# daigo0927/tf-raft

Measured on NVIDIA H100. Metric: frame-pairs/sec at 448×512 iters=12; final-flow max-abs vs ref, higher is better.
Workload: dtype f32

## Files before the change

tf_raft_b200/csrc/conv_tc.cuh:

```cuda
#pragma once
#include "common.cuh"
#include "kernels.cuh"
#include "tmap.cuh"

namespace raft {

enum TcEpilogue : int {
  EPI_LINEAR = 0,
  EPI_GRU_ZR = 1,
  EPI_GRU_Q = 2,
};
enum TcAct : int { ACT_NONE = 0, ACT_RELU = 1 };

constexpr int kTileM = 128;
constexpr int kChunkK = 64;
constexpr int kABytes = kTileM * kChunkK * 2;
constexpr int kMaxTileN = 128;
constexpr int kConsumerWGs = 2;
constexpr int kConsumerWarps = 4 * kConsumerWGs;
constexpr int kTcThreads = 128 * kConsumerWGs + 128;
constexpr int kStageCols = 64;
constexpr int kStagingBytes = kConsumerWGs * 64 * kStageCols * 4;
constexpr int kSmemMax = 227 * 1024;
constexpr int kSmemFixed = 1024  + kStagingBytes + 512 ;

struct alignas(64) TcConvParams {
  CUtensorMap a_map[2];
  CUtensorMap b_map;
  int nseg, seg_chunks[2], seg_c0[2];
  int kh, kw, ph, pw;
  int stride;
  int B, H, W, TH, TW, tiles_x, tiles_y;
  int bn, n_total;
  int n_tiles_n;
  int nstages, stage_bytes;
  int group_chunks;
  int mode, act;
  const float* bias;
  const float* inv_scale;
  float out_scale;
  float* out_f32; int f32_stride, f32_c0;
  __half* out_hi; __half* out_lo; int h_stride, h_c0;
  const float* post_scale;
  const float* post_shift;
  const float* residual; int res_stride, res_c0;
  const float* concat_src; int concat_n;
  float* z; int hid;
  float* h;
  float* adv_coords;
  float* adv_flow;
};

#if defined(__CUDA_ARCH__)
__device__ __forceinline__ float4 ld4(const float* p) { return *reinterpret_cast<const float4*>(p); }
__device__ __forceinline__ float4 ldg4(const float* p) { return __ldg(reinterpret_cast<const float4*>(p)); }
__device__ __forceinline__ void st4(float* p, float4 v) { *reinterpret_cast<float4*>(p) = v; }
__device__ __forceinline__ void st8u(void* p, const uint32_t (&r)[8]) {
  reinterpret_cast<uint4*>(p)[0] = make_uint4(r[0], r[1], r[2], r[3]);
  reinterpret_cast<uint4*>(p)[1] = make_uint4(r[4], r[5], r[6], r[7]);
}
__device__ __forceinline__ void ldcg8(const float* p, float (&r)[8]) {
  const float4 a = __ldcg(reinterpret_cast<const float4*>(p)), b = __ldcg(reinterpret_cast<const float4*>(p) + 1);
  r[0] = a.x; r[1] = a.y; r[2] = a.z; r[3] = a.w; r[4] = b.x; r[5] = b.y; r[6] = b.z; r[7] = b.w;
}
__device__ __forceinline__ void ldnc8(const float* p, float (&r)[8]) {
  const float4 a = __ldg(reinterpret_cast<const float4*>(p)), b = __ldg(reinterpret_cast<const float4*>(p) + 1);
  r[0] = a.x; r[1] = a.y; r[2] = a.z; r[3] = a.w; r[4] = b.x; r[5] = b.y; r[6] = b.z; r[7] = b.w;
}
__device__ __forceinline__ void st8f(float* p, float a, float b, float c, float d, float e, float f, float g, float h) {
  const uint32_t r[8] = {__float_as_uint(a), __float_as_uint(b), __float_as_uint(c), __float_as_uint(d),
                         __float_as_uint(e), __float_as_uint(f), __float_as_uint(g), __float_as_uint(h)};
  st8u(p, r);
}
__device__ __forceinline__ float4 ldcg4(const float* p) { return __ldcg(reinterpret_cast<const float4*>(p)); }

__device__ __forceinline__ float fast_sigmoid(float x) { return __fdividef(1.0f, 1.0f + __expf(-x)); }
__device__ __forceinline__ float fast_tanh(float x) { return 1.0f - __fdividef(2.0f, 1.0f + __expf(2.0f * x)); }

template <int MODE>
__device__ __forceinline__ void tc_epilogue_regs(const TcConvParams& p, float (&v)[32], size_t pix, int col, int ncol,
                                                 float inv_scale) {
  if (p.bias) {
#pragma unroll
    for (int q = 0; q < 8; ++q) {
      const float4 bq = ldg4(p.bias + col + 4 * q);
      v[4 * q] = v[4 * q] * inv_scale + bq.x; v[4 * q + 1] = v[4 * q + 1] * inv_scale + bq.y;
      v[4 * q + 2] = v[4 * q + 2] * inv_scale + bq.z; v[4 * q + 3] = v[4 * q + 3] * inv_scale + bq.w;
    }
  } else {
#pragma unroll
    for (int j = 0; j < 32; ++j) v[j] *= inv_scale;
  }
  if (MODE == EPI_LINEAR && p.post_scale) {
#pragma unroll
    for (int q = 0; q < 8; ++q) {
      const float4 sc = ldg4(p.post_scale + col + 4 * q), sh = ldg4(p.post_shift + col + 4 * q);
      v[4 * q] = v[4 * q] * sc.x + sh.x; v[4 * q + 1] = v[4 * q + 1] * sc.y + sh.y;
      v[4 * q + 2] = v[4 * q + 2] * sc.z + sh.z; v[4 * q + 3] = v[4 * q + 3] * sc.w + sh.w;
    }
  }

  __half* dhi = nullptr;
  __half* dlo = nullptr;
  if (MODE == EPI_LINEAR) {
    const bool full = col + 32 <= p.n_total;
// ... 119 lines not shown

  if (dhi) {
    const bool wide = ((reinterpret_cast<uintptr_t>(dhi) | reinterpret_cast<uintptr_t>(dlo)) & 31) == 0;
#pragma unroll
    for (int q = 0; q < 2; ++q) {
      uint32_t ph[8], pl[8];
#pragma unroll
      for (int e = 0; e < 8; ++e) split_f16x2(v[16 * q + 2 * e], v[16 * q + 2 * e + 1], ph[e], pl[e]);
      if (wide) {
        st8u(dhi + 16 * q, ph);
        st8u(dlo + 16 * q, pl);
      } else {
        reinterpret_cast<uint4*>(dhi)[2 * q] = make_uint4(ph[0], ph[1], ph[2], ph[3]);
        reinterpret_cast<uint4*>(dhi)[2 * q + 1] = make_uint4(ph[4], ph[5], ph[6], ph[7]);
        reinterpret_cast<uint4*>(dlo)[2 * q] = make_uint4(pl[0], pl[1], pl[2], pl[3]);
        reinterpret_cast<uint4*>(dlo)[2 * q + 1] = make_uint4(pl[4], pl[5], pl[6], pl[7]);
      }
    }
  }
}

struct RingPos {
  int slot;
  uint32_t par;
};

__device__ __forceinline__ int ring_next(RingPos& r, int nst) {
  const int s = r.slot;
  r.slot = s + 1 == nst ? 0 : s + 1;
  return s;
}

__device__ __forceinline__ void ring_init(uint64_t* full_bar, uint64_t* empty_bar, int nst) {
  for (int s = 0; s < nst; ++s) {
    mbar_init(&full_bar[s], 1);
    mbar_init(&empty_bar[s], kConsumerWarps);
  }
}

struct RingSlot {
  uint8_t* data;
  uint64_t* full;
};

__device__ __forceinline__ RingSlot ring_acquire(uint8_t* stages, const int& slot_bytes, const int& nst, uint64_t* full_bar,
                                                 uint64_t* empty_bar, RingPos& rp, const int& tx) {
  const int s = ring_next(rp, nst);
  mbar_wait(&empty_bar[s], ((rp.par >> s) & 1u) ^ 1u);
  rp.par ^= 1u << s;
  mbar_arrive_expect_tx(&full_bar[s], (uint32_t)tx);
  return RingSlot{stages + (size_t)s * slot_bytes, &full_bar[s]};
}

template <int N>
__device__ __forceinline__ void ring_mma(float (&racc)[N / 2], uint8_t* stages, const int& slot_bytes, const int& nst,
                                         uint64_t* full_bar, uint64_t* empty_bar, RingPos& rp, int wg, uint32_t b_lo_off,
                                         int total, const int& group_chunks) {
  const int lane = threadIdx.x & 31;
  float acc[N / 2];
#pragma unroll
  for (int i = 0; i < N / 2; ++i) acc[i] = racc[i] = 0.0f;
  for (int done = 0; done < total;) {
    const int gend = min(total, done + group_chunks);
    for (int first = 1; done < gend; ++done, first = 0) {
      const int s = ring_next(rp, nst);
      mbar_wait(&full_bar[s], (rp.par >> s) & 1u);
      rp.par ^= 1u << s;
      const uint32_t sa = smem_u32(stages + (size_t)s * slot_bytes);
      const uint32_t arow = (uint32_t)wg * 64 * 128;
      wgmma_fence_regs(acc);
      wgmma_fence();
      wgmma_chunk3<N>(acc, make_desc_sw128(sa + arow), make_desc_sw128(sa + kABytes + arow), make_desc_sw128(sa + 2 * kABytes),
                      make_desc_sw128(sa + 2 * kABytes + b_lo_off), first != 0);
      wgmma_commit();
      wgmma_wait_all();
      wgmma_fence_regs(acc);
      __syncwarp();
      if (lane == 0) mbar_arrive(&empty_bar[s]);
    }
#pragma unroll
    for (int i = 0; i < N / 2; ++i) racc[i] += acc[i];
  }
}

__device__ __forceinline__ int tc_total_chunks(const TcConvParams& c) {
  return c.kh * c.kw * (c.seg_chunks[0] + (c.nseg > 1 ? c.seg_chunks[1] : 0));
}

__device__ __forceinline__ void tc_produce_tile(const TcConvParams& c, uint8_t* stages, uint64_t* full_bar, uint64_t* empty_bar,
                                                RingPos& rp, int nt, int b, int ty, int tx, unsigned int* next_item = nullptr,
                                                int* claim = nullptr) {
  const int ntaps = c.kh * c.kw;
  const int x0 = tx * c.TW * c.stride, y0 = ty * c.TH * c.stride, n0 = nt * c.bn;
  int left = tc_total_chunks(c);
  for (int tap = 0; tap < ntaps; ++tap) {
    const int dy = tap / c.kw - c.ph, dx = tap % c.kw - c.pw;
    int kc = 0;
    for (int seg = 0; seg < c.nseg; ++seg) {
      for (int ch = 0; ch < c.seg_chunks[seg]; ++ch, ++kc) {
        if (--left == 0 && claim) *claim = (int)atomicAdd(next_item, 1u);
        const RingSlot st = ring_acquire(stages, c.stage_bytes, c.nstages, full_bar, empty_bar, rp, c.stage_bytes);
        tma_load_5d(st.data, &c.a_map[seg], st.full, c.seg_c0[seg] + ch * kChunkK, x0 + dx, y0 + dy, b, 0);
        tma_load_4d(st.data + 2 * kABytes, &c.b_map, st.full, kc * kChunkK, n0, tap, 0);
      }
    }
  }
}

__device__ __forceinline__ int stg_idx(int r, int c) { return r * kStageCols + ((((c >> 2) ^ (r & 7))) << 2) + (c & 3); }

template <int N>
__device__ __forceinline__ void tc_consume_tile(const TcConvParams& c, uint8_t* stages, float* staging, uint64_t* full_bar,
                                                uint64_t* empty_bar, RingPos& rp, int wg, int tid, int nt, int b, int ty,
                                                int tx) {
  const int lane = tid & 31, w = tid >> 5;
  float racc[N / 2];
  ring_mma<N>(racc, stages, c.stage_bytes, c.nstages, full_bar, empty_bar, rp, wg, (uint32_t)(c.bn * kChunkK * 2),
              tc_total_chunks(c), c.group_chunks);

  float* stg = staging + wg * 64 * kStageCols;
  const int row = tid & 63, half = tid >> 6;
  const int m = wg * 64 + row;
  const int x = tx * c.TW + m % c.TW, y = ty * c.TH + m / c.TW;
  const bool inside = x < c.W && y < c.H;
  const size_t pix = ((size_t)b * c.H + y) * c.W + x;
  const float inv_scale = c.inv_scale ? __ldg(c.inv_scale) : 1.0f;
#pragma unroll
  for (int cb = 0; cb < (N + kStageCols - 1) / kStageCols; ++cb) {
    if (cb * kStageCols >= c.bn) break;
    wg_sync(wg);
#pragma unroll
    for (int i = cb * 8; i < min(cb * 8 + 8, N / 8); ++i) {
      const int col = 8 * (i - cb * 8) + 2 * (lane & 3), r0 = 16 * w + (lane >> 2);
      *reinterpret_cast<float2*>(stg + stg_idx(r0, col)) = make_float2(racc[4 * i], racc[4 * i + 1]);
      *reinterpret_cast<float2*>(stg + stg_idx(r0 + 8, col)) = make_float2(racc[4 * i + 2], racc[4 * i + 3]);
    }
    wg_sync(wg);
    const int c0 = cb * kStageCols + half * 32;
    if (inside && c0 < c.bn) {
      const int ncol = min(32, c.bn - c0);
      float v[32];
#pragma unroll
      for (int q = 0; q < 8; ++q) {
        const float4 t4 = *reinterpret_cast<const float4*>(stg + stg_idx(row, half * 32 + 4 * q));
        v[4 * q] = t4.x; v[4 * q + 1] = t4.y; v[4 * q + 2] = t4.z; v[4 * q + 3] = t4.w;
      }
#pragma unroll
      for (int j = 0; j < 32; ++j)
        if (j >= ncol) v[j] = 0.0f;
      if (c.mode == EPI_LINEAR) tc_epilogue_regs<EPI_LINEAR>(c, v, pix, nt * c.bn + c0, ncol, inv_scale);
      else if (c.mode == EPI_GRU_ZR) tc_epilogue_regs<EPI_GRU_ZR>(c, v, pix, nt * c.bn + c0, ncol, inv_scale);
      else tc_epilogue_regs<EPI_GRU_Q>(c, v, pix, nt * c.bn + c0, ncol, inv_scale);
    }
  }
}

template <class F>
__device__ __forceinline__ void with_mma_n(int bn, F&& f) {
  if (bn <= 16) f(std::integral_constant<int, 16>{});
  else if (bn <= 32) f(std::integral_constant<int, 32>{});
  else if (bn <= 64) f(std::integral_constant<int, 64>{});
  else if (bn <= 96) f(std::integral_constant<int, 96>{});
  else f(std::integral_constant<int, 128>{});
}

__device__ __forceinline__ void regs_producer() { asm volatile("setmaxnreg.dec.sync.aligned.u32 40;\n" ::: "memory"); }
__device__ __forceinline__ void regs_consumer() { asm volatile("setmaxnreg.inc.sync.aligned.u32 232;\n" ::: "memory"); }

__device__ __forceinline__ void tc_decode_tile(const TcConvParams& c, int t, int& nt, int& b, int& ty, int& tx) {
  const int mtiles = c.B * c.tiles_y * c.tiles_x;
  nt = t / mtiles;
  int mt = t - nt * mtiles;
  tx = mt % c.tiles_x;
  mt /= c.tiles_x;
  ty = mt % c.tiles_y;
  b = mt / c.tiles_y;
}
#endif

__global__ void __launch_bounds__(kTcThreads, 1) conv_tc_kernel(const __grid_constant__ TcConvParams p) {
#if defined(__CUDA_ARCH__)
  extern __shared__ uint8_t smem_raw[];
  uint8_t* smem = reinterpret_cast<uint8_t*>((reinterpret_cast<uintptr_t>(smem_raw) + 1023) & ~uintptr_t(1023));
  const int nst = p.nstages;
  uint8_t* stages = smem;
  float* staging = reinterpret_cast<float*>(stages + (size_t)nst * p.stage_bytes);
  uint64_t* full_bar = reinterpret_cast<uint64_t*>(reinterpret_cast<uint8_t*>(staging) + kStagingBytes);
  uint64_t* empty_bar = full_bar + nst;

  const int warp = threadIdx.x >> 5;
  const int mtiles = p.B * p.tiles_y * p.tiles_x;
  const int ntiles = mtiles * p.n_tiles_n;

  if (threadIdx.x == 0) {
    ring_init(full_bar, empty_bar, nst);
    fence_mbar_init();
  }
  if (warp == kConsumerWarps && (threadIdx.x & 31) == 0) {
    prefetch_tmap(&p.a_map[0]);
    prefetch_tmap(&p.b_map);
    if (p.nseg > 1) prefetch_tmap(&p.a_map[1]);
  }
  __syncthreads();
  asm volatile("griddepcontrol.wait;" ::: "memory");
  asm volatile("griddepcontrol.launch_dependents;" ::: "memory");

  RingPos rp{0, 0u};
  if (warp >= kConsumerWarps) {
    regs_producer();
    if (warp == kConsumerWarps && elect_one()) {
      for (int t = blockIdx.x; t < ntiles; t += gridDim.x) {
        int nt, b, ty, tx;
        tc_decode_tile(p, t, nt, b, ty, tx);
        tc_produce_tile(p, stages, full_bar, empty_bar, rp, nt, b, ty, tx);
      }
    }
  } else {
    regs_consumer();
    const int wg = warp >> 2, tid = threadIdx.x & 127;
    with_mma_n(p.bn, [&](auto n) {
      for (int t = blockIdx.x; t < ntiles; t += gridDim.x) {
        int nt, b, ty, tx;
        tc_decode_tile(p, t, nt, b, ty, tx);
        tc_consume_tile<decltype(n)::value>(p, stages, staging, full_bar, empty_bar, rp, wg, tid, nt, b, ty, tx);
      }
    });
  }
#endif
}

inline void tc_pick_tile(int W, int H, int* tw, int* th) {
  long best = -1;
  for (int t = 128; t >= 8; t >>= 1) {
    const int hh = 128 / t;
    const long area = (long)round_up(W, t) * round_up(H, hh);
    if (best < 0 || area < best) {
      best = area;
      *tw = t;
      *th = hh;
    }
  }
}

inline int tc_n_split(int bn) {
  const int f = ceil_div(bn, kMaxTileN);
  return bn % (16 * f) == 0 ? f : 0;
}

inline int tc_finalize(TcConvParams& p) {
  p.tiles_x = ceil_div(p.W, p.TW);
  p.tiles_y = ceil_div(p.H, p.TH);
  p.stage_bytes = 2 * kABytes + 2 * p.bn * kChunkK * 2;
  int nst = (kSmemMax - kSmemFixed) / p.stage_bytes;
  if (nst > 8) nst = 8;
  p.nstages = nst;
  return nst * p.stage_bytes + kSmemFixed;
}

inline int tc_check(const TcConvParams& p) {
  if (p.bn % 16 != 0 || p.bn < 16 || p.bn > kMaxTileN || p.TW * p.TH != kTileM) return RAFT_ERR_BAD_SHAPE;
  if (p.mode != EPI_LINEAR && p.mode != EPI_GRU_ZR && p.mode != EPI_GRU_Q) return RAFT_ERR_UNSUPPORTED;
  if (p.group_chunks < 1) return RAFT_ERR_BAD_ARG;
  return RAFT_OK;
}

template <auto Kernel>
inline int persistent_grid(int smem, long items, unsigned* grid) {
  static int num_sms[64] = {0};
  int dev = 0;
  RAFT_CUDA_TRY(cudaGetDevice(&dev));
  int& sms = num_sms[dev & 63];
  if (!sms) {
    RAFT_CUDA_TRY(cudaFuncSetAttribute(Kernel, cudaFuncAttributeMaxDynamicSharedMemorySize, smem));
    RAFT_CUDA_TRY(cudaDeviceGetAttribute(&sms, cudaDevAttrMultiProcessorCount, dev));
  }
  *grid = (unsigned)(items < sms ? items : sms);
  return RAFT_OK;
}

inline int tc_launch(TcConvParams& p, int n_tiles_n, cudaStream_t stream) {
  RAFT_TRY(tc_check(p));
  if (p.stride < 1) p.stride = 1;
  const int smem = tc_finalize(p);
  if (p.nstages < 2) return RAFT_ERR_UNSUPPORTED;
  p.n_tiles_n = n_tiles_n;
  unsigned grid = 0;
  RAFT_TRY(persistent_grid<conv_tc_kernel>(kSmemMax, (long)p.B * p.tiles_y * p.tiles_x * n_tiles_n, &grid));
  cudaLaunchConfig_t cfg;
  memset(&cfg, 0, sizeof(cfg));
  cfg.gridDim = dim3(grid);
  cfg.blockDim = dim3((unsigned)kTcThreads);
  cfg.dynamicSmemBytes = (size_t)smem;
  cfg.stream = stream;
  cudaLaunchAttribute attr[1];
  attr[0].id = cudaLaunchAttributeProgrammaticStreamSerialization;
  attr[0].val.programmaticStreamSerializationAllowed = 1;
  cfg.attrs = attr;
  cfg.numAttrs = 1;
  ++g_launches;
  RAFT_CUDA_TRY(cudaLaunchKernelEx(&cfg, conv_tc_kernel, p));
  return raft_launch_status();
}

struct TcWeightSlot {
  size_t hi, lo, bias, scale, absmax;
  int kh, kw, cin_pad, cout_pad;
};

inline TcWeightSlot tc_weight_slot(size_t& off, int kh, int kw, int cin_pad, int cout_pad) {
  auto take = [&](size_t bytes) { const size_t o = off; off = align_up(off + bytes, 256); return o; };
  TcWeightSlot s;
  s.kh = kh; s.kw = kw; s.cin_pad = cin_pad; s.cout_pad = cout_pad;
  const size_t plane = (size_t)kh * kw * cout_pad * cin_pad * sizeof(__half);
  s.hi = take(plane);
  s.lo = take(plane);
// ... 56 lines not shown
```

tf_raft_b200/csrc/encoder.cuh:

```cuda
#pragma once
#include <algorithm>

#include "lookup.cuh"
#include "update.cuh"

namespace raft {

enum { NORM_NONE = 0, NORM_INSTANCE = 1, NORM_BATCH = 2 };

struct EncSpec { int c0; int c[3]; int s[3]; };
inline EncSpec enc_spec(int variant) {
  if (variant == RAFT_VARIANT_BASIC) return {64, {64, 96, 128}, {1, 2, 2}};
  return {32, {32, 64, 96}, {1, 2, 2}};
}
inline int pad64(int c) { return round_up(c, 64); }

struct EncNormSlot { size_t gamma, beta, fscale, fshift; int C; };
struct EncLayout {
  TcWeightSlot conv1;
  EncNormSlot norm1;
  TcWeightSlot bc1[6], bc2[6], bds[6];
  EncNormSlot bn1[6], bn2[6], bnd[6];
  int has_ds[6], bc[6], bstride[6];
  TcWeightSlot conv2;
// ... 12 lines not shown
    n.C = C;
    n.gamma = take(sizeof(float) * (C + 64)); n.beta = take(sizeof(float) * (C + 64));
    n.fscale = take(sizeof(float) * (C + 64)); n.fshift = take(sizeof(float) * (C + 64));
    return n;
  };
  L.conv1 = conv_slot(1, 1, 147, S.c0);
  L.norm1 = norm_slot(S.c0);
  int cin = S.c0;
  for (int k = 0; k < 6; ++k) {
    const int c = S.c[k / 2], st = (k % 2 == 0) ? S.s[k / 2] : 1;
    L.bc[k] = c; L.bstride[k] = st;
    L.bc1[k] = conv_slot(3, 3, cin, c);
    L.bc2[k] = conv_slot(3, 3, c, c);
    L.bn1[k] = norm_slot(c);
    L.bn2[k] = norm_slot(c);
    L.has_ds[k] = st != 1;
    if (L.has_ds[k]) { L.bds[k] = conv_slot(1, 1, cin, c); L.bnd[k] = norm_slot(c); }
    cin = c;
  }
  L.conv2 = conv_slot(1, 1, cin, out_dim);
  L.total = off;
  return L;
}

struct EncWs {
  float *X32, *O32, *Y32, *D32;
  __half *Xh, *Xl, *Oh, *Ol, *Fh, *Fl, *Ih, *Il;
  float *part, *mean, *mult;
  size_t total;
};
constexpr int kNormSplit = 64;
inline EncWs enc_ws_layout(void* base, int variant, int N, int H, int W) {
  EncWs E;
  memset(&E, 0, sizeof(E));
  const EncSpec S = enc_spec(variant);
  size_t max32 = 0, max16 = 0;
  for (int l = 0; l < 3; ++l) {
    const int d = 2 << l;
    const size_t np = (size_t)N * ((H + d - 1) / d) * ((W + d - 1) / d);
    const int c = l == 0 ? (S.c0 > S.c[0] ? S.c0 : S.c[0]) : S.c[l];
    if (np * c > max32) max32 = np * c;
    if (np * pad64(c) > max16) max16 = np * pad64(c);
  }
  uint8_t* b8 = reinterpret_cast<uint8_t*>(base);
  size_t off = 0;
  auto take = [&](size_t bytes) { uint8_t* p = b8 + off; off = align_up(off + bytes, 1024); return p; };
  E.X32 = (float*)take(max32 * 4); E.O32 = (float*)take(max32 * 4);
  E.Y32 = (float*)take(max32 * 4); E.D32 = (float*)take(max32 * 4);
  E.Xh = (__half*)take(max16 * 2); E.Xl = (__half*)take(max16 * 2);
  E.Oh = (__half*)take(max16 * 2); E.Ol = (__half*)take(max16 * 2);
  E.Fh = (__half*)take(max16 * 2); E.Fl = (__half*)take(max16 * 2);
  {
    const size_t np1 = (size_t)N * ((H + 1) / 2) * ((W + 1) / 2);
    E.Ih = (__half*)take(np1 * 192 * 2); E.Il = (__half*)take(np1 * 192 * 2);
  }
  E.part = (float*)take((size_t)N * kNormSplit * 3 * 256 * 4);
  E.mean = (float*)take((size_t)N * 256 * 4);
  E.mult = (float*)take((size_t)N * 256 * 4);
  E.total = off;
  return E;
}

inline int enc_pack_conv(const raft_conv& cv, int kh, int kw, int cin, int cout, const TcWeightSlot& s, bool flatten,
                         uint8_t* base, cudaStream_t st) {
  if (!cv.kernel || !cv.bias) return RAFT_ERR_BAD_ARG;
  if (cv.kh != kh || cv.kw != kw || cv.cin != cin || cv.cout != cout) return RAFT_ERR_BAD_SHAPE;
  const raft_conv* src[1] = {&cv};
  return tc_pack_weights(base, s, src, 1, nullptr, flatten, st);
}

inline int enc_pack_norm(const raft_norm& nm, const EncNormSlot& s, int norm_type, uint8_t* base, cudaStream_t st) {
  if (norm_type == NORM_NONE) return 0;
  if (!nm.gamma || !nm.beta) return RAFT_ERR_BAD_ARG;
  float* g = reinterpret_cast<float*>(base + s.gamma);
  float* b = reinterpret_cast<float*>(base + s.beta);
  RAFT_CUDA_TRY(cudaMemcpyAsync(g, nm.gamma, s.C * sizeof(float), cudaMemcpyDeviceToDevice, st));
  RAFT_CUDA_TRY(cudaMemcpyAsync(b, nm.beta, s.C * sizeof(float), cudaMemcpyDeviceToDevice, st));
  if (norm_type == NORM_BATCH) {
    if (!nm.moving_mean || !nm.moving_variance) return RAFT_ERR_BAD_ARG;
    return launch(bn_fold_kernel, ceil_div(s.C, 128), 128, 0, st, nm.gamma, nm.beta, nm.moving_mean, nm.moving_variance,
                  1e-3f, s.C, reinterpret_cast<float*>(base + s.fscale), reinterpret_cast<float*>(base + s.fshift));
  }
  return raft_launch_status();
}

inline int encoder_prepare(int variant, int norm_type, int out_dim, const raft_encoder_weights* w, void* prepared,
                           size_t bytes, cudaStream_t st) {
  const EncLayout L = enc_layout(variant, out_dim);
  if (L.total > bytes) return RAFT_ERR_WORKSPACE;
  const EncSpec S = enc_spec(variant);
  uint8_t* base = reinterpret_cast<uint8_t*>(prepared);
  RAFT_CUDA_TRY(cudaMemsetAsync(base, 0, L.total, st));
  RAFT_TRY(enc_pack_conv(w->conv1, 7, 7, 3, S.c0, L.conv1, true, base, st));
  RAFT_TRY(enc_pack_norm(w->norm1, L.norm1, norm_type, base, st));
  int cin = S.c0;
  for (int k = 0; k < 6; ++k) {
    const int c = L.bc[k];
    RAFT_TRY(enc_pack_conv(w->block[k].conv1, 3, 3, cin, c, L.bc1[k], false, base, st));
    RAFT_TRY(enc_pack_conv(w->block[k].conv2, 3, 3, c, c, L.bc2[k], false, base, st));
    RAFT_TRY(enc_pack_norm(w->block[k].norm1, L.bn1[k], norm_type, base, st));
    RAFT_TRY(enc_pack_norm(w->block[k].norm2, L.bn2[k], norm_type, base, st));
    if (L.has_ds[k]) {
      RAFT_TRY(enc_pack_conv(w->block[k].downsample, 1, 1, cin, c, L.bds[k], false, base, st));
      RAFT_TRY(enc_pack_norm(w->block[k].downsample_norm, L.bnd[k], norm_type, base, st));
    }
    cin = c;
  }
  RAFT_TRY(enc_pack_conv(w->conv2, 1, 1, cin, out_dim, L.conv2, false, base, st));
  return raft_launch_status();
}

struct EncCtx {
  const uint8_t* prep; EncLayout L; EncWs W; cudaStream_t st;
  int N, norm_type, stats;
  int per_image;
};

inline int enc_norm_apply(const EncCtx& c, const EncNormSlot& ns, const float* y, size_t npix, int P, int relu,
                          const float* skip32, const __half* skip_hi, const __half* skip_lo, float* out32, __half* hi,
                          __half* lo) {
  const int C = ns.C, G = c.per_image ? c.N : 1;
  const int Pg = c.per_image ? P : (int)npix;
  const float* gamma = reinterpret_cast<const float*>(c.prep + ns.gamma);
  const float* beta = reinterpret_cast<const float*>(c.prep + ns.beta);
  RAFT_TRY(launch(norm_stats_kernel, dim3((unsigned)G, kNormSplit), 256, 0, c.st, y, Pg, C, kNormSplit, c.W.part));
  RAFT_TRY(launch(norm_final_kernel, ceil_div(G * C * 32, 256), 256, 0, c.st, c.W.part, G, C, kNormSplit, gamma, 1e-3f,
                  c.W.mean, c.W.mult));
  return launch(norm_apply_kernel, grid_for(npix * (pad64(C) / 8)), 256, 0, c.st, y, npix, P, C, c.per_image, c.W.mean,
                c.W.mult, beta, relu, skip32, skip_hi, skip_lo, out32, hi, lo, pad64(C));
}

inline int enc_conv_tc(const EncCtx& c, const TcWeightSlot& cs, int cout, const EncNormSlot* ns, const __half* ahi,
                       const __half* alo, int Hin, int Win, int Hout, int Wout, int stride, int relu, const float* skip,
                       float* out32, __half* ohi, __half* olo) {
  TcConvParams p;
  memset(&p, 0, sizeof(p));
  int tw, th;
  tc_pick_tile(Wout, Hout, &tw, &th);
  if (tw * stride > 256) tw = 128 / stride, th = 128 / tw;
  const int nsplit = tc_n_split(cs.cout_pad);
  if (!nsplit) return RAFT_ERR_BAD_SHAPE;
  RAFT_TRY(make_tmap_act2(&p.a_map[0], ahi, alo, c.N, Hin, Win, cs.cin_pad, tw, th, stride));
  RAFT_TRY(tc_use_weights(p, c.prep, cs, cs.cout_pad / nsplit));
  p.nseg = 1; p.seg_chunks[0] = cs.cin_pad / kChunkK; p.seg_c0[0] = 0;
  p.stride = stride;
  if (stride == 1) { p.ph = (cs.kh - 1) / 2; p.pw = (cs.kw - 1) / 2; }
  else {
    const int tot_h = (Hout - 1) * stride + cs.kh - Hin, tot_w = (Wout - 1) * stride + cs.kw - Win;
    p.ph = (tot_h > 0 ? tot_h : 0) / 2; p.pw = (tot_w > 0 ? tot_w : 0) / 2;
  }
  p.B = c.N; p.H = Hout; p.W = Wout; p.TH = th; p.TW = tw;
  p.n_total = cout;
  p.mode = EPI_LINEAR; p.out_scale = 1.0f;
  p.out_f32 = out32; p.f32_stride = cout; p.f32_c0 = 0;
  p.out_hi = ohi; p.out_lo = olo; p.h_stride = pad64(cout); p.h_c0 = 0;
  if (ns && !c.stats && c.norm_type == NORM_BATCH) {
    p.post_scale = reinterpret_cast<const float*>(c.prep + ns->fscale);
    p.post_shift = reinterpret_cast<const float*>(c.prep + ns->fshift);
  }
  const bool fused = !(ns && c.stats);
  if (fused) {
    p.act = relu ? ACT_RELU : ACT_NONE;
    p.residual = skip; p.res_stride = cout; p.res_c0 = 0;
  } else {
    p.act = ACT_NONE; p.out_hi = nullptr; p.out_lo = nullptr;
  }
  p.group_chunks = 5;
  return tc_launch(p, nsplit, c.st);
}

inline int encoder_forward(int variant, int norm_type, int out_dim, const void* prepared, const float* images, int N,
                           int H, int W, int training, int image_norm, float* out, void* ws, size_t ws_bytes, cudaStream_t st) {
  EncCtx c;
  c.prep = reinterpret_cast<const uint8_t*>(prepared);
  c.L = enc_layout(variant, out_dim);
  c.W = enc_ws_layout(ws, variant, N, H, W);
  if (c.W.total > ws_bytes) return RAFT_ERR_WORKSPACE;
  c.st = st; c.N = N; c.norm_type = norm_type;
  c.stats = (norm_type == NORM_INSTANCE) || (norm_type == NORM_BATCH && training);
  c.per_image = norm_type == NORM_INSTANCE;
  const EncSpec S = enc_spec(variant);
  const EncLayout& L = c.L;
  const EncWs& E = c.W;

  int h = (H + 1) / 2, w = (W + 1) / 2;
  {
    const size_t npix = (size_t)N * h * w;
    const int tot_h = (h - 1) * 2 + 7 - H, tot_w = (w - 1) * 2 + 7 - W;
    const float* src = images;
    if (image_norm) {
      const size_t nimg = (size_t)N * H * W * 3;
      RAFT_TRY(launch(image_norm_kernel, grid_for(nimg), 256, 0, st, images, E.O32, nimg));
      src = E.O32;
    }
    RAFT_TRY(launch(stem_im2col_kernel, grid_for(npix * 24), 256, 0, st, src, N, H, W, h, w, (tot_h > 0 ? tot_h : 0) / 2,
                    (tot_w > 0 ? tot_w : 0) / 2, 0, E.Ih, E.Il));
    if (!c.stats && pad64(S.c0) != S.c0) {
      RAFT_CUDA_TRY(cudaMemsetAsync(E.Xh, 0, npix * pad64(S.c0) * 2, st));
      RAFT_CUDA_TRY(cudaMemsetAsync(E.Xl, 0, npix * pad64(S.c0) * 2, st));
    }
    RAFT_TRY(enc_conv_tc(c, L.conv1, S.c0, &L.norm1, E.Ih, E.Il, h, w, h, w, 1, 1, nullptr, c.stats ? E.Y32 : E.X32, E.Xh, E.Xl));
    if (c.stats) RAFT_TRY(enc_norm_apply(c, L.norm1, E.Y32, npix, h * w, 1, nullptr, nullptr, nullptr, nullptr, E.Xh, E.Xl));
  }

  float *X32 = E.X32, *O32 = E.O32;
  __half *Xh = E.Xh, *Xl = E.Xl, *Oh = E.Oh, *Ol = E.Ol;
  for (int k = 0; k < 6; ++k) {
    const int st2 = L.bstride[k], cc = L.bc[k];
    const int ho = (h + st2 - 1) / st2, wo = (w + st2 - 1) / st2;
    const size_t npo = (size_t)N * ho * wo;
    const bool zero_pad_out = pad64(cc) != cc;
    if (!c.stats && zero_pad_out) {
      RAFT_CUDA_TRY(cudaMemsetAsync(E.Fh, 0, npo * pad64(cc) * 2, st));
      RAFT_CUDA_TRY(cudaMemsetAsync(E.Fl, 0, npo * pad64(cc) * 2, st));
      RAFT_CUDA_TRY(cudaMemsetAsync(Oh, 0, npo * pad64(cc) * 2, st));
      RAFT_CUDA_TRY(cudaMemsetAsync(Ol, 0, npo * pad64(cc) * 2, st));
    }
    RAFT_TRY(enc_conv_tc(c, L.bc1[k], cc, &L.bn1[k], Xh, Xl, h, w, ho, wo, st2, 1, nullptr, c.stats ? E.Y32 : nullptr, E.Fh, E.Fl));
    if (c.stats) RAFT_TRY(enc_norm_apply(c, L.bn1[k], E.Y32, npo, ho * wo, 1, nullptr, nullptr, nullptr, nullptr, E.Fh, E.Fl));
    const float* skip = X32;
    if (L.has_ds[k]) {
      RAFT_TRY(enc_conv_tc(c, L.bds[k], cc, &L.bnd[k], Xh, Xl, h, w, ho, wo, st2, 0, nullptr, c.stats ? E.Y32 : E.D32, nullptr, nullptr));
      if (c.stats) RAFT_TRY(enc_norm_apply(c, L.bnd[k], E.Y32, npo, ho * wo, 0, nullptr, nullptr, nullptr, E.D32, nullptr, nullptr));
      skip = E.D32;
    }
    RAFT_TRY(enc_conv_tc(c, L.bc2[k], cc, &L.bn2[k], E.Fh, E.Fl, ho, wo, ho, wo, 1, 1, skip, c.stats ? E.Y32 : O32, Oh, Ol));
    if (c.stats) {
      if (L.has_ds[k]) RAFT_TRY(enc_norm_apply(c, L.bn2[k], E.Y32, npo, ho * wo, 1, E.D32, nullptr, nullptr, nullptr, Oh, Ol));
      else RAFT_TRY(enc_norm_apply(c, L.bn2[k], E.Y32, npo, ho * wo, 1, nullptr, Xh, Xl, nullptr, Oh, Ol));
    }
    float* t32 = X32; X32 = O32; O32 = t32;
    __half* th_ = Xh; Xh = Oh; Oh = th_;
    __half* tl_ = Xl; Xl = Ol; Ol = tl_;
    h = ho; w = wo;
  }
  RAFT_TRY(enc_conv_tc(c, L.conv2, out_dim, nullptr, Xh, Xl, h, w, h, w, 1, 0, nullptr, out, nullptr, nullptr));
  return raft_launch_status();
}

}
```

tf_raft_b200/csrc/kernels.cuh:

```cuda
#pragma once
#include "common.cuh"

namespace raft {

__global__ void split_plane_kernel(const float* __restrict__ src, int src_stride, int src_c0, int nch, int nch_pad,
                                   __half* __restrict__ hi, __half* __restrict__ lo, int dst_stride, int dst_c0,
                                   size_t npix, float scale) {
  const size_t total = npix * (size_t)nch_pad;
  for (size_t i = blockIdx.x * (size_t)blockDim.x + threadIdx.x; i < total; i += (size_t)gridDim.x * blockDim.x) {
    const size_t px = i / nch_pad;
    const int c = (int)(i - px * nch_pad);
    __half h = __float2half_rn(0.f), l = h;
    if (c < nch) split_f16(src[px * src_stride + src_c0 + c] * scale, h, l);
    hi[px * dst_stride + dst_c0 + c] = h;
    lo[px * dst_stride + dst_c0 + c] = l;
  }
}

__global__ void avgpool2x2_kernel(const float* __restrict__ src, float* __restrict__ dst, size_t M, int H, int W,
                                  int C) {
  const int Ho = H / 2, Wo = W / 2;
  const size_t total = M * (size_t)Ho * Wo * C;
  for (size_t i = blockIdx.x * (size_t)blockDim.x + threadIdx.x; i < total; i += (size_t)gridDim.x * blockDim.x) {
    size_t t = i;
// ... 511 lines not shown
  const size_t total = npix * (size_t)gpp;
  for (size_t i = blockIdx.x * (size_t)blockDim.x + threadIdx.x; i < total; i += (size_t)gridDim.x * blockDim.x) {
    const size_t px = i / gpp;
    const int c = (int)(i - px * gpp) << 3;
    float v[8] = {0.f, 0.f, 0.f, 0.f, 0.f, 0.f, 0.f, 0.f};
    if (c < C) {
      const size_t g = per_image ? px / P : 0;
      const float* yp = y + px * C + c;
      const float* mp = mean + g * C + c;
      const float* ap = a + g * C + c;
      const float* bp = beta + c;
      float4 t[2] = {*reinterpret_cast<const float4*>(yp), *reinterpret_cast<const float4*>(yp + 4)};
      const float yy[8] = {t[0].x, t[0].y, t[0].z, t[0].w, t[1].x, t[1].y, t[1].z, t[1].w};
#pragma unroll
      for (int e = 0; e < 8; ++e) {
        v[e] = (yy[e] - __ldg(mp + e)) * __ldg(ap + e) + __ldg(bp + e);
        if (relu) v[e] = relu_nan(v[e]);
      }
      if (skip32) {
        const float4 s0 = *reinterpret_cast<const float4*>(skip32 + px * C + c), s1 = *reinterpret_cast<const float4*>(skip32 + px * C + c + 4);
        const float ss[8] = {s0.x, s0.y, s0.z, s0.w, s1.x, s1.y, s1.z, s1.w};
#pragma unroll
        for (int e = 0; e < 8; ++e) v[e] = relu_nan(ss[e] + v[e]);
      } else if (skip_hi) {
        const uint4 h4 = *reinterpret_cast<const uint4*>(skip_hi + px * c_pad + c), l4 = *reinterpret_cast<const uint4*>(skip_lo + px * c_pad + c);
        const uint32_t hw[4] = {h4.x, h4.y, h4.z, h4.w}, lw[4] = {l4.x, l4.y, l4.z, l4.w};
#pragma unroll
        for (int e = 0; e < 4; ++e) {
          const float2 hf = __half22float2(*reinterpret_cast<const __half2*>(&hw[e]));
          const float2 lf = __half22float2(*reinterpret_cast<const __half2*>(&lw[e]));
          v[2 * e] = relu_nan(hf.x + lf.x + v[2 * e]);
          v[2 * e + 1] = relu_nan(hf.y + lf.y + v[2 * e + 1]);
        }
      }
      if (out32) {
        *reinterpret_cast<float4*>(out32 + px * C + c) = make_float4(v[0], v[1], v[2], v[3]);
        *reinterpret_cast<float4*>(out32 + px * C + c + 4) = make_float4(v[4], v[5], v[6], v[7]);
      }
    }
    if (hi) {
      uint32_t ph[4], pl[4];
#pragma unroll
      for (int e = 0; e < 4; ++e) split_f16x2(v[2 * e], v[2 * e + 1], ph[e], pl[e]);
      *reinterpret_cast<uint4*>(hi + px * c_pad + c) = make_uint4(ph[0], ph[1], ph[2], ph[3]);
      *reinterpret_cast<uint4*>(lo + px * c_pad + c) = make_uint4(pl[0], pl[1], pl[2], pl[3]);
    }
  }
}
__global__ void image_norm_kernel(const float* __restrict__ img, float* __restrict__ out, size_t n) {
  for (size_t i = blockIdx.x * (size_t)blockDim.x + threadIdx.x; i < n; i += (size_t)gridDim.x * blockDim.x)
    out[i] = __fsub_rn(__fmul_rn(2.0f, __fdiv_rn(img[i], 255.0f)), 1.0f);
}

__global__ void stem_im2col_kernel(const float* __restrict__ img, int N, int H, int W, int h, int w, int pad_t,
                                   int pad_l, int image_norm, __half* __restrict__ hi, __half* __restrict__ lo) {
  const size_t total = (size_t)N * h * w * 24;
  for (size_t i = blockIdx.x * (size_t)blockDim.x + threadIdx.x; i < total; i += (size_t)gridDim.x * blockDim.x) {
    const int grp = (int)(i % 24);
    const size_t px = i / 24;
    const int x = (int)(px % w), y = (int)((px / w) % h), n = (int)(px / ((size_t)w * h));
    uint32_t ph[4] = {0u, 0u, 0u, 0u}, pl[4] = {0u, 0u, 0u, 0u};
    if (grp * 8 < 147) {
      int ty = (grp * 8) / 21, j = grp * 8 - ty * 21;
      const int ix0 = 2 * x - pad_l;
      const float* base = img + ((size_t)n * H * W + ix0) * 3;
      float v[8];
#pragma unroll
      for (int e = 0; e < 8; ++e) {
        const int iy = 2 * y + ty - pad_t, ix = ix0 + ((j * 11) >> 5);
        v[e] = 0.f;
        if (ty < 7 && iy >= 0 && iy < H && ix >= 0 && ix < W) {
          v[e] = __ldg(base + (ptrdiff_t)iy * W * 3 + j);
          if (image_norm) v[e] = __fsub_rn(__fmul_rn(2.0f, __fdiv_rn(v[e], 255.0f)), 1.0f);
        }
        if (++j == 21) { j = 0; ++ty; }
      }
#pragma unroll
      for (int e = 0; e < 4; ++e) split_f16x2(v[2 * e], v[2 * e + 1], ph[e], pl[e]);
    }
    reinterpret_cast<uint4*>(hi)[i] = make_uint4(ph[0], ph[1], ph[2], ph[3]);
    reinterpret_cast<uint4*>(lo)[i] = make_uint4(pl[0], pl[1], pl[2], pl[3]);
  }
}

__device__ __forceinline__ void flow_im2col_rider(const float* __restrict__ flow, int B, int h, int w, __half* __restrict__ hi,
                                                  __half* __restrict__ lo, size_t tid, size_t nthreads) {
  const size_t total = (size_t)B * h * w * 16;
  for (size_t i = tid; i < total; i += nthreads) {
    const int g = (int)(i & 15);
    const size_t px = i >> 4;
    const int x = (int)(px % w), y = (int)((px / w) % h);
    uint32_t ph[4], pl[4];
#pragma unroll
    for (int e = 0; e < 4; ++e) {
      const int tap = 4 * g + e;
      float2 v = make_float2(0.f, 0.f);
      if (tap < 49) {
        const int yy = y + tap / 7 - 3, xx = x + tap % 7 - 3;
        if (yy >= 0 && yy < h && xx >= 0 && xx < w)
          v = __ldg(reinterpret_cast<const float2*>(flow) + (ptrdiff_t)px + (ptrdiff_t)(yy - y) * w + (xx - x));
      }
      split_f16x2(v.x, v.y, ph[e], pl[e]);
    }
    reinterpret_cast<uint4*>(hi)[i] = make_uint4(ph[0], ph[1], ph[2], ph[3]);
    reinterpret_cast<uint4*>(lo)[i] = make_uint4(pl[0], pl[1], pl[2], pl[3]);
  }
}

__global__ void flow_im2col_kernel(const float* __restrict__ flow, int B, int h, int w, __half* __restrict__ hi,
                                   __half* __restrict__ lo) {
  const size_t total = (size_t)B * h * w * 128;
  for (size_t i = blockIdx.x * (size_t)blockDim.x + threadIdx.x; i < total; i += (size_t)gridDim.x * blockDim.x) {
// ... 47 lines not shown
```

Before: 262.7.

## Load 3x3 conv input halo once per tile and index taps from shared memory

Adds a halo mode to the tensor-core conv for stride-1 3x3 encoder convs with 64 input channels. Each output tile loads one padded input patch (hi and lo planes) into shared memory, and per-tap WGMMA descriptors point at offsets inside it, so the input is no longer fetched by TMA once per tap. Only the weights go through the ring, and the next tile's halo is prefetched. Separately, the stem im2col buffer is narrowed from 192 to 152 channels to cut write traffic, with the A tensor map told the real channel count. The halo path relies on hand-built shared-memory descriptor layouts, and the padded tail chunk of the stem's K dimension must still hold valid data.

```diff
diff --git a/tf_raft_b200/csrc/conv_tc.cuh b/tf_raft_b200/csrc/conv_tc.cuh
--- a/tf_raft_b200/csrc/conv_tc.cuh
+++ b/tf_raft_b200/csrc/conv_tc.cuh
@@ -34,6 +34,7 @@
   int bn, n_total;
   int n_tiles_n;
   int nstages, stage_bytes;
+  int halo;
   int group_chunks;
   int mode, act;
   const float* bias;
@@ -51,6 +52,21 @@
   float* adv_flow;
 };
 
+constexpr int kHaloTW = 64, kHaloTH = 2;
+constexpr int kHaloW = kHaloTW + 2, kHaloH = kHaloTH + 2;
+constexpr int kHaloPlaneBytes = kHaloW * kHaloH * 128;
+constexpr int kHaloBytes = 2 * kHaloPlaneBytes;
+
+__host__ __device__ inline uint64_t tc_halo_desc(uint32_t halo, int plane, int w, int ky, int kx) {
+  const uint32_t start = halo + (uint32_t)plane * kHaloPlaneBytes + (uint32_t)(((w + ky) * kHaloW + kx) * 128);
+  uint64_t d = 0;
+  d |= (uint64_t)((start & 0x3FFFF) >> 4);
+  d |= (uint64_t)1 << 16;
+  d |= (uint64_t)(1024 >> 4) << 32;
+  d |= (uint64_t)1 << 62;
+  return d;
+}
+
 #if defined(__CUDA_ARCH__)
 __device__ __forceinline__ float4 ld4(const float* p) { return *reinterpret_cast<const float4*>(p); }
 __device__ __forceinline__ float4 ldg4(const float* p) { return __ldg(reinterpret_cast<const float4*>(p)); }
@@ -276,10 +292,10 @@
   return RingSlot{stages + (size_t)s * slot_bytes, &full_bar[s]};
 }
 
-template <int N>
-__device__ __forceinline__ void ring_mma(float (&racc)[N / 2], uint8_t* stages, const int& slot_bytes, const int& nst,
-                                         uint64_t* full_bar, uint64_t* empty_bar, RingPos& rp, int wg, uint32_t b_lo_off,
-                                         int total, const int& group_chunks) {
+template <int N, class ADesc>
+__device__ __forceinline__ void ring_mma_a(float (&racc)[N / 2], uint8_t* stages, const int& slot_bytes, const int& nst,
+                                           uint64_t* full_bar, uint64_t* empty_bar, RingPos& rp, uint32_t b_off,
+                                           uint32_t b_lo_off, int total, const int& group_chunks, ADesc&& a_desc) {
   const int lane = threadIdx.x & 31;
   float acc[N / 2];
 #pragma unroll
@@ -291,11 +307,11 @@
       mbar_wait(&full_bar[s], (rp.par >> s) & 1u);
       rp.par ^= 1u << s;
       const uint32_t sa = smem_u32(stages + (size_t)s * slot_bytes);
-      const uint32_t arow = (uint32_t)wg * 64 * 128;
+      uint64_t a_hi, a_lo;
+      a_desc(sa, done, a_hi, a_lo);
       wgmma_fence_regs(acc);
       wgmma_fence();
-      wgmma_chunk3<N>(acc, make_desc_sw128(sa + arow), make_desc_sw128(sa + kABytes + arow), make_desc_sw128(sa + 2 * kABytes),
-                      make_desc_sw128(sa + 2 * kABytes + b_lo_off), first != 0);
+      wgmma_chunk3<N>(acc, a_hi, a_lo, make_desc_sw128(sa + b_off), make_desc_sw128(sa + b_off + b_lo_off), first != 0);
       wgmma_commit();
       wgmma_wait_all();
       wgmma_fence_regs(acc);
@@ -305,6 +321,18 @@
 #pragma unroll
     for (int i = 0; i < N / 2; ++i) racc[i] += acc[i];
   }
+}
+
+template <int N>
+__device__ __forceinline__ void ring_mma(float (&racc)[N / 2], uint8_t* stages, const int& slot_bytes, const int& nst,
+                                         uint64_t* full_bar, uint64_t* empty_bar, RingPos& rp, int wg, uint32_t b_lo_off,
+                                         int total, const int& group_chunks) {
+  ring_mma_a<N>(racc, stages, slot_bytes, nst, full_bar, empty_bar, rp, 2 * kABytes, b_lo_off, total, group_chunks,
+                [wg](uint32_t sa, int, uint64_t& a_hi, uint64_t& a_lo) {
+                  const uint32_t arow = (uint32_t)wg * 64 * 128;
+                  a_hi = make_desc_sw128(sa + arow);
+                  a_lo = make_desc_sw128(sa + kABytes + arow);
+                });
 }
 
 __device__ __forceinline__ int tc_total_chunks(const TcConvParams& c) {
@@ -331,17 +359,19 @@
   }
 }
 
+__device__ __forceinline__ void tc_load_halo(const TcConvParams& c, uint8_t* halo, uint64_t* hfull, uint64_t* hempty, int j,
+                                             int b, int ty, int tx) {
+  mbar_wait(hempty, (j & 1) ^ 1);
+  mbar_arrive_expect_tx(hfull, (uint32_t)kHaloBytes);
+  tma_load_5d(halo, &c.a_map[0], hfull, 0, tx * kHaloTW - c.pw, ty * kHaloTH - c.ph, b, 0);
+}
+
 __device__ __forceinline__ int stg_idx(int r, int c) { return r * kStageCols + ((((c >> 2) ^ (r & 7))) << 2) + (c & 3); }
 
 template <int N>
-__device__ __forceinline__ void tc_consume_tile(const TcConvParams& c, uint8_t* stages, float* staging, uint64_t* full_bar,
-                                                uint64_t* empty_bar, RingPos& rp, int wg, int tid, int nt, int b, int ty,
-                                                int tx) {
+__device__ __forceinline__ void tc_epilogue_tile(const TcConvParams& c, const float (&racc)[N / 2], float* staging, int wg,
+                                                 int tid, int nt, int b, int ty, int tx) {
   const int lane = tid & 31, w = tid >> 5;
-  float racc[N / 2];
-  ring_mma<N>(racc, stages, c.stage_bytes, c.nstages, full_bar, empty_bar, rp, wg, (uint32_t)(c.bn * kChunkK * 2),
-              tc_total_chunks(c), c.group_chunks);
-
   float* stg = staging + wg * 64 * kStageCols;
   const int row = tid & 63, half = tid >> 6;
   const int m = wg * 64 + row;
@@ -377,6 +407,34 @@
       else tc_epilogue_regs<EPI_GRU_Q>(c, v, pix, nt * c.bn + c0, ncol, inv_scale);
     }
   }
+}
+
+template <int N>
+__device__ __forceinline__ void tc_consume_tile(const TcConvParams& c, uint8_t* stages, float* staging, uint64_t* full_bar,
+                                                uint64_t* empty_bar, RingPos& rp, int wg, int tid, int nt, int b, int ty,
+                                                int tx) {
+  float racc[N / 2];
+  ring_mma<N>(racc, stages, c.stage_bytes, c.nstages, full_bar, empty_bar, rp, wg, (uint32_t)(c.bn * kChunkK * 2),
+              tc_total_chunks(c), c.group_chunks);
+  tc_epilogue_tile<N>(c, racc, staging, wg, tid, nt, b, ty, tx);
+}
+
+template <int N>
+__device__ __forceinline__ void tc_consume_tile_halo(const TcConvParams& c, uint8_t* halo, uint64_t* hfull, uint64_t* hempty,
+                                                     int j, uint8_t* stages, float* staging, uint64_t* full_bar,
+                                                     uint64_t* empty_bar, RingPos& rp, int wg, int tid, int nt, int b,
+                                                     int ty, int tx) {
+  mbar_wait(hfull, j & 1);
+  const uint32_t hbase = smem_u32(halo);
+  float racc[N / 2];
+  ring_mma_a<N>(racc, stages, c.stage_bytes, c.nstages, full_bar, empty_bar, rp, 0u, (uint32_t)(c.bn * kChunkK * 2),
+                c.kh * c.kw, c.group_chunks, [hbase, wg](uint32_t, int tap, uint64_t& a_hi, uint64_t& a_lo) {
+                  a_hi = tc_halo_desc(hbase, 0, wg, tap / 3, tap % 3);
+                  a_lo = tc_halo_desc(hbase, 1, wg, tap / 3, tap % 3);
+                });
+  __syncwarp();
+  if ((tid & 31) == 0) mbar_arrive(hempty);
+  tc_epilogue_tile<N>(c, racc, staging, wg, tid, nt, b, ty, tx);
 }
 
 template <class F>
@@ -407,10 +465,13 @@
   extern __shared__ uint8_t smem_raw[];
   uint8_t* smem = reinterpret_cast<uint8_t*>((reinterpret_cast<uintptr_t>(smem_raw) + 1023) & ~uintptr_t(1023));
   const int nst = p.nstages;
-  uint8_t* stages = smem;
+  uint8_t* halo = smem;
+  uint8_t* stages = smem + (p.halo ? kHaloBytes : 0);
   float* staging = reinterpret_cast<float*>(stages + (size_t)nst * p.stage_bytes);
   uint64_t* full_bar = reinterpret_cast<uint64_t*>(reinterpret_cast<uint8_t*>(staging) + kStagingBytes);
   uint64_t* empty_bar = full_bar + nst;
+  uint64_t* hfull = empty_bar + nst;
+  uint64_t* hempty = hfull + 1;
 
   const int warp = threadIdx.x >> 5;
   const int mtiles = p.B * p.tiles_y * p.tiles_x;
@@ -418,6 +479,7 @@
 
   if (threadIdx.x == 0) {
     ring_init(full_bar, empty_bar, nst);
+    ring_init(hfull, hempty, 1);
     fence_mbar_init();
   }
   if (warp == kConsumerWarps && (threadIdx.x & 31) == 0) {
@@ -433,20 +495,44 @@
   if (warp >= kConsumerWarps) {
     regs_producer();
     if (warp == kConsumerWarps && elect_one()) {
-      for (int t = blockIdx.x; t < ntiles; t += gridDim.x) {
+      if (p.halo) {
         int nt, b, ty, tx;
-        tc_decode_tile(p, t, nt, b, ty, tx);
-        tc_produce_tile(p, stages, full_bar, empty_bar, rp, nt, b, ty, tx);
+        if (blockIdx.x < ntiles) {
+          tc_decode_tile(p, blockIdx.x, nt, b, ty, tx);
+          tc_load_halo(p, halo, hfull, hempty, 0, b, ty, tx);
+        }
+        for (int t = blockIdx.x, j = 0; t < ntiles; t += gridDim.x, ++j) {
+          tc_decode_tile(p, t, nt, b, ty, tx);
+          for (int tap = 0; tap < p.kh * p.kw; ++tap) {
+            const RingSlot st = ring_acquire(stages, p.stage_bytes, p.nstages, full_bar, empty_bar, rp, p.stage_bytes);
+            tma_load_4d(st.data, &p.b_map, st.full, 0, nt * p.bn, tap, 0);
+            if (tap == p.kh * p.kw - 1 && t + (int)gridDim.x < ntiles) {
+              int nt1, b1, ty1, tx1;
+              tc_decode_tile(p, t + gridDim.x, nt1, b1, ty1, tx1);
+              tc_load_halo(p, halo, hfull, hempty, j + 1, b1, ty1, tx1);
+            }
+          }
+        }
+      } else {
+        for (int t = blockIdx.x; t < ntiles; t += gridDim.x) {
+          int nt, b, ty, tx;
+          tc_decode_tile(p, t, nt, b, ty, tx);
+          tc_produce_tile(p, stages, full_bar, empty_bar, rp, nt, b, ty, tx);
+        }
       }
     }
   } else {
     regs_consumer();
     const int wg = warp >> 2, tid = threadIdx.x & 127;
     with_mma_n(p.bn, [&](auto n) {
-      for (int t = blockIdx.x; t < ntiles; t += gridDim.x) {
+      for (int t = blockIdx.x, j = 0; t < ntiles; t += gridDim.x, ++j) {
         int nt, b, ty, tx;
         tc_decode_tile(p, t, nt, b, ty, tx);
-        tc_consume_tile<decltype(n)::value>(p, stages, staging, full_bar, empty_bar, rp, wg, tid, nt, b, ty, tx);
+        if (p.halo)
+          tc_consume_tile_halo<decltype(n)::value>(p, halo, hfull, hempty, j, stages, staging, full_bar, empty_bar, rp, wg,
+                                                   tid, nt, b, ty, tx);
+        else
+          tc_consume_tile<decltype(n)::value>(p, stages, staging, full_bar, empty_bar, rp, wg, tid, nt, b, ty, tx);
       }
     });
   }
@@ -474,17 +560,21 @@
 inline int tc_finalize(TcConvParams& p) {
   p.tiles_x = ceil_div(p.W, p.TW);
   p.tiles_y = ceil_div(p.H, p.TH);
-  p.stage_bytes = 2 * kABytes + 2 * p.bn * kChunkK * 2;
-  int nst = (kSmemMax - kSmemFixed) / p.stage_bytes;
+  const int fixed = kSmemFixed + (p.halo ? kHaloBytes : 0);
+  p.stage_bytes = (p.halo ? 0 : 2 * kABytes) + 2 * p.bn * kChunkK * 2;
+  int nst = (kSmemMax - fixed) / p.stage_bytes;
   if (nst > 8) nst = 8;
   p.nstages = nst;
-  return nst * p.stage_bytes + kSmemFixed;
+  return nst * p.stage_bytes + fixed;
 }
 
 inline int tc_check(const TcConvParams& p) {
   if (p.bn % 16 != 0 || p.bn < 16 || p.bn > kMaxTileN || p.TW * p.TH != kTileM) return RAFT_ERR_BAD_SHAPE;
   if (p.mode != EPI_LINEAR && p.mode != EPI_GRU_ZR && p.mode != EPI_GRU_Q) return RAFT_ERR_UNSUPPORTED;
   if (p.group_chunks < 1) return RAFT_ERR_BAD_ARG;
+  if (p.halo && (p.kh != 3 || p.kw != 3 || p.stride != 1 || p.nseg != 1 || p.seg_chunks[0] != 1 || p.TW != kHaloTW ||
+                 p.TH != kHaloTH))
+    return RAFT_ERR_BAD_SHAPE;
   return RAFT_OK;
 }
 
diff --git a/tf_raft_b200/csrc/encoder.cuh b/tf_raft_b200/csrc/encoder.cuh
--- a/tf_raft_b200/csrc/encoder.cuh
+++ b/tf_raft_b200/csrc/encoder.cuh
@@ -88,7 +88,7 @@
   E.Fh = (__half*)take(max16 * 2); E.Fl = (__half*)take(max16 * 2);
   {
     const size_t np1 = (size_t)N * ((H + 1) / 2) * ((W + 1) / 2);
-    E.Ih = (__half*)take(np1 * 192 * 2); E.Il = (__half*)take(np1 * 192 * 2);
+    E.Ih = (__half*)take(np1 * kStemC * 2); E.Il = (__half*)take(np1 * kStemC * 2);
   }
   E.part = (float*)take((size_t)N * kNormSplit * 3 * 256 * 4);
   E.mean = (float*)take((size_t)N * 256 * 4);
@@ -166,9 +166,14 @@
                 c.W.mult, beta, relu, skip32, skip_hi, skip_lo, out32, hi, lo, pad64(C));
 }
 
+inline bool enc_halo_enabled() {
+  static const int v = [] { const char* e = getenv("RAFT_B200_ENC_HALO"); return e ? atoi(e) : 1; }();
+  return v != 0;
+}
+
 inline int enc_conv_tc(const EncCtx& c, const TcWeightSlot& cs, int cout, const EncNormSlot* ns, const __half* ahi,
                        const __half* alo, int Hin, int Win, int Hout, int Wout, int stride, int relu, const float* skip,
-                       float* out32, __half* ohi, __half* olo) {
+                       float* out32, __half* ohi, __half* olo, int a_channels = 0) {
   TcConvParams p;
   memset(&p, 0, sizeof(p));
   int tw, th;
@@ -176,7 +181,13 @@
   if (tw * stride > 256) tw = 128 / stride, th = 128 / tw;
   const int nsplit = tc_n_split(cs.cout_pad);
   if (!nsplit) return RAFT_ERR_BAD_SHAPE;
-  RAFT_TRY(make_tmap_act2(&p.a_map[0], ahi, alo, c.N, Hin, Win, cs.cin_pad, tw, th, stride));
+  p.halo = enc_halo_enabled() && stride == 1 && cs.kh == 3 && cs.kw == 3 && cs.cin_pad == kChunkK && cs.cout_pad <= 64;
+  if (p.halo) {
+    tw = kHaloTW; th = kHaloTH;
+    RAFT_TRY(make_tmap_act2(&p.a_map[0], ahi, alo, c.N, Hin, Win, cs.cin_pad, kHaloW, kHaloH));
+  } else {
+    RAFT_TRY(make_tmap_act2(&p.a_map[0], ahi, alo, c.N, Hin, Win, a_channels ? a_channels : cs.cin_pad, tw, th, stride));
+  }
   RAFT_TRY(tc_use_weights(p, c.prep, cs, cs.cout_pad / nsplit));
   p.nseg = 1; p.seg_chunks[0] = cs.cin_pad / kChunkK; p.seg_c0[0] = 0;
   p.stride = stride;
@@ -229,13 +240,14 @@
       RAFT_TRY(launch(image_norm_kernel, grid_for(nimg), 256, 0, st, images, E.O32, nimg));
       src = E.O32;
     }
-    RAFT_TRY(launch(stem_im2col_kernel, grid_for(npix * 24), 256, 0, st, src, N, H, W, h, w, (tot_h > 0 ? tot_h : 0) / 2,
+    RAFT_TRY(launch(stem_im2col_kernel, grid_for(npix * (kStemC / 8)), 256, 0, st, src, N, H, W, h, w, (tot_h > 0 ? tot_h : 0) / 2,
                     (tot_w > 0 ? tot_w : 0) / 2, 0, E.Ih, E.Il));
     if (!c.stats && pad64(S.c0) != S.c0) {
       RAFT_CUDA_TRY(cudaMemsetAsync(E.Xh, 0, npix * pad64(S.c0) * 2, st));
       RAFT_CUDA_TRY(cudaMemsetAsync(E.Xl, 0, npix * pad64(S.c0) * 2, st));
     }
-    RAFT_TRY(enc_conv_tc(c, L.conv1, S.c0, &L.norm1, E.Ih, E.Il, h, w, h, w, 1, 1, nullptr, c.stats ? E.Y32 : E.X32, E.Xh, E.Xl));
+    RAFT_TRY(enc_conv_tc(c, L.conv1, S.c0, &L.norm1, E.Ih, E.Il, h, w, h, w, 1, 1, nullptr, c.stats ? E.Y32 : E.X32, E.Xh, E.Xl,
+                         kStemC));
     if (c.stats) RAFT_TRY(enc_norm_apply(c, L.norm1, E.Y32, npix, h * w, 1, nullptr, nullptr, nullptr, nullptr, E.Xh, E.Xl));
   }
 
diff --git a/tf_raft_b200/csrc/kernels.cuh b/tf_raft_b200/csrc/kernels.cuh
--- a/tf_raft_b200/csrc/kernels.cuh
+++ b/tf_raft_b200/csrc/kernels.cuh
@@ -587,12 +587,14 @@
     out[i] = __fsub_rn(__fmul_rn(2.0f, __fdiv_rn(img[i], 255.0f)), 1.0f);
 }
 
+constexpr int kStemC = 152;
 __global__ void stem_im2col_kernel(const float* __restrict__ img, int N, int H, int W, int h, int w, int pad_t,
                                    int pad_l, int image_norm, __half* __restrict__ hi, __half* __restrict__ lo) {
-  const size_t total = (size_t)N * h * w * 24;
-  for (size_t i = blockIdx.x * (size_t)blockDim.x + threadIdx.x; i < total; i += (size_t)gridDim.x * blockDim.x) {
-    const int grp = (int)(i % 24);
-    const size_t px = i / 24;
+  constexpr int G = kStemC / 8;
+  const size_t total = (size_t)N * h * w * G;
+  for (size_t i = blockIdx.x * (size_t)blockDim.x + threadIdx.x; i < total; i += (size_t)gridDim.x * blockDim.x) {
+    const int grp = (int)(i % G);
+    const size_t px = i / G;
     const int x = (int)(px % w), y = (int)((px / w) % h), n = (int)(px / ((size_t)w * h));
     uint32_t ph[4] = {0u, 0u, 0u, 0u}, pl[4] = {0u, 0u, 0u, 0u};
     if (grp * 8 < 147) {
```

Result: no change. 264.2, median of 6 (+0.5%).
